# Kingsford-Group/squid

Hardware: AMD Instinct MI355X
Metric: paired-end alignments/sec BAM->_sv.txt (from the BAM files in the page cache: file read, host->device copy, BGZF/BAM decode, graph, ordering, SV calls, _sv.txt written; bit-exact SV calls vs CPU oracle) (higher is better)
Workload: dtype int32

## Files before the change

squid_amd/csrc/sq_inflate_spec.inc:

```
#pragma once
#include "sq_wave.h"

#ifndef SQ_SPEC_PRE
#define SQ_SPEC_PRE 0
#endif
namespace isp {
#ifdef SQ_WAVE_EMU
struct EmuStat { unsigned long long iters = 0, pairs = 0, lits = 0, matches = 0, stretches = 0, max_iters_sum = 0;
    unsigned long long windows = 0, rounds = 0, wave_steps_fix = 0, wave_steps_emit = 0, lane_steps_fix = 0; uint32_t ls[2][64] = {}, le[64] = {};
    void round_done(int par) { uint32_t m = 0; for (int i = 0; i < 64; ++i) { m = ls[par][i] > m ? ls[par][i] : m; lane_steps_fix += ls[par][i]; ls[par][i] = 0; } wave_steps_fix += m; ++rounds; }
    void emit_done() { uint32_t m = 0; for (int i = 0; i < 64; ++i) { m = le[i] > m ? le[i] : m; le[i] = 0; } wave_steps_emit += m; ++windows; } };
inline EmuStat& emu_stat() { static EmuStat s; return s; }
inline int& emu_par_of(int lane) { static int p[64] = {}; return p[lane]; }
#define emu_par() emu_par_of(wv::lane())
#define ISP_STAT(x) x
#else
#define ISP_STAT(x)
#endif

constexpr uint32_t E_VAL = 8, E_XOFF = 17, E_XB = 24, E_NL = 28, E_LIT1 = 1u << 28, E_LIT2 = 2u << 28, E_MATCH = 1u << 30, E_SUB = 1u << 31;
template <int PB> struct Enough;
template <> struct Enough<9> { static constexpr int LL = 852; };
template <> struct Enough<10> { static constexpr int LL = 1334; };
template <> struct Enough<11> { static constexpr int LL = 2342; };
constexpr int DD_PB = 8, DD_N = 402;
constexpr uint32_t OUT_EOB = 1u << 30, OUT_BAD = 1u << 31, OUT_POS = (1u << 30) - 1;

template <int CH, int PB>
struct Lay {
    static constexpr int LL_N = Enough<PB>::LL;
    static constexpr int WIN_DW = (64 * CH / 32 + 16 < 368 ? 368 : 64 * CH / 32 + 16);
    static constexpr int WIN = 0, LENS = WIN, LL = WIN_DW, DD = LL + ((LL_N + 3) & ~3), CLT = DD, MISC = DD + ((DD_N + 3) & ~3), END = MISC + 16;
    static constexpr int BYTES = END * 4;
};
static inline __host__ __device__ uint32_t tok_cap_spec(uint32_t isize, uint32_t clen) { return ((isize >> 1) + (clen >> 3) + 256u + 3u) & ~3u; }

struct Src { const uint32_t* w; uint32_t lim_dw; };
WV_FN uint32_t src_ld(const Src& s, uint32_t d) { return d < s.lim_dw ? s.w[d] : 0u; }
WV_FN unsigned long long src_peek64(const Src& s, uint32_t pos) {
    const uint32_t d = pos >> 5, w0 = src_ld(s, d), w1 = src_ld(s, d + 1), w2 = src_ld(s, d + 2);
    return ((unsigned long long)wv::alignbit(w2, w1, pos) << 32) | wv::alignbit(w1, w0, pos);
}
WV_FN uint32_t ll_entry(int sym, int len) {
    if (sym < 256) return (uint32_t)len | E_LIT1 | ((uint32_t)sym << E_VAL);
    if (sym == 256) return (uint32_t)len;
    const int ls = sym - 257;
    if (ls >= 29) return 0u;
    const uint32_t lx = ls < 8 || ls == 28 ? 0u : (uint32_t)(ls - 4) >> 2;
    const uint32_t lbase = ls < 8 ? 3u + (uint32_t)ls : (ls == 28 ? 258u : 3u + ((4u + ((uint32_t)ls & 3u)) << lx));
    return ((uint32_t)len + lx) | (lbase << E_VAL) | (((uint32_t)len + 2u) << E_XOFF) | (lx << E_XB) | E_MATCH;
}
WV_FN uint32_t dd_entry(int sym, int len) {
    if (sym >= 30) return 0u;
    const uint32_t dx = sym < 4 ? 0u : (uint32_t)(sym - 2) >> 1;
    const uint32_t dbase = sym < 4 ? 1u + (uint32_t)sym : 1u + ((2u + ((uint32_t)sym & 1u)) << dx);
    return ((uint32_t)len + dx) | (dbase << E_VAL) | (dx << E_XB);
}

template <bool IS_LL, int PBITS, int N, int ROUNDS>
WV_FN bool build_table(wv::lds_u32* tbl, const wv::lds_u8* lens, int nsym, wv::lds_u32* alloc_word) {
    const int lane = wv::lane();
    for (int q = lane; q < N; q += 64) tbl[q] = 0u;
    if (lane == 0) *alloc_word = 0u;
    int mylen[ROUNDS];
    uint32_t cnt[16];
#pragma unroll
    for (int l = 0; l < 16; ++l) cnt[l] = 0;
#pragma unroll
// ... 58 lines not shown
        for (int r = 0; r < ROUNDS; ++r) {
            const int l = mylen[r];
            if (l > PBITS) {
                const uint32_t rv = mycode[r], link = tbl[rv & ((1u << PBITS) - 1u)];
                if (link & E_SUB) {
                    const uint32_t nb = (link >> E_XB) & 15u, base = ((link >> E_VAL) & 0xffffu) >> 2;
                    const uint32_t ent = IS_LL ? ll_entry(r * 64 + lane, l) : dd_entry(r * 64 + lane, l);
                    for (uint32_t k = rv >> PBITS; k < (1u << nb); k += 1u << (l - PBITS)) tbl[base + k] = ent;
                }
            }
        }
        wv::sync();
        if (wv::any(!ok)) return false;
    }
    if (IS_LL) {
        for (int i = lane; i < (1 << PBITS); i += 64) {
            const uint32_t e1 = tbl[i];
            if ((e1 >> E_NL) == 1u) {
                const uint32_t cl1 = e1 & 0xffu;
                if (cl1 < (uint32_t)PBITS) {
                    const uint32_t e2 = tbl[(uint32_t)i >> cl1], nl2 = (e2 >> E_NL) & 3u;
                    if (nl2 && !(e2 & (E_SUB | E_MATCH))) {
                        const uint32_t cl2 = nl2 == 2u ? (e2 >> E_XB) & 15u : e2 & 0xffu;
                        if (cl1 + cl2 <= (uint32_t)PBITS) tbl[i] = (cl1 + cl2) | (((e1 >> E_VAL) & 0xffu) << E_VAL) | (((e2 >> E_VAL) & 0xffu) << (E_VAL + 8)) | (cl1 << E_XB) | E_LIT2;
                    }
                }
            }
        }
        wv::sync();
    }
    return true;
}

template <int MODE, int PB>
WV_FN void scan_stretch(const wv::lds_u8* ll, const wv::lds_u8* dd, const wv::lds_u8* win_q , uint32_t start, uint32_t lim,
                        uint32_t* tk , uint32_t at , uint32_t& out, uint32_t& ntok) {
    uint32_t q = start - 2u, nt = at, lit = 0, nlit = 0, status = 0;
    const uint32_t limq = lim - 2u;
    while (q < limq) {
        const wv::lds_u8* wp = win_q + ((q >> 5) << 2);
        const uint32_t w0 = *(const wv::lds_u32*)wp, w1 = *(const wv::lds_u32*)(wp + 4), w2 = *(const wv::lds_u32*)(wp + 8);
        const uint32_t lo = wv::alignbit(w1, w0, q);
        uint32_t e = *(const wv::lds_u32*)(ll + (lo & (((1u << PB) - 1u) << 2)));
        if ((int32_t)e < 0) e = *(const wv::lds_u32*)(ll + ((e >> E_VAL) & 0xffffu) + (wv::bfe(lo, PB + 2, (e >> E_XB) & 15u) << 2));
        const uint32_t nl = (e >> E_NL) & 3u, tot = e & 0xffu, q0 = q;
        ISP_STAT(if (MODE == 2) { ++emu_stat().iters; emu_stat().lits += nl; emu_stat().pairs += nl == 2; emu_stat().matches += e >= E_MATCH; ++emu_stat().le[wv::lane()]; } else ++emu_stat().ls[emu_par()][wv::lane()];)
        q += tot;
        if (MODE) {
            if (MODE == 2) lit |= (nl ? (e >> E_VAL) & 0xffffu : 0u) << (8u * nlit);
            nlit += nl;
            if (nlit >= 3u) {
                if (MODE == 2) { tk[nt] = (lit & 0xffffffu) | (3u << 24); lit >>= 24; }
                ++nt; nlit -= 3u;
            }
        }
        if (e >= E_MATCH) {
            if (MODE) { if (nlit) { if (MODE == 2) { tk[nt] = lit | (nlit << 24); lit = 0; } ++nt; nlit = 0; } }
            const uint32_t hi = wv::alignbit(w2, w1, q0);
            const unsigned long long rest = (((unsigned long long)hi << 32) | lo) >> tot;
            const uint32_t rlo = (uint32_t)rest;
            uint32_t d = *(const wv::lds_u32*)(dd + (rlo & (((1u << DD_PB) - 1u) << 2)));
            if ((int32_t)d < 0) d = *(const wv::lds_u32*)(dd + ((d >> E_VAL) & 0xffffu) + (wv::bfe(rlo, DD_PB + 2, (d >> E_XB) & 15u) << 2));
            if (d == 0u) { status = OUT_BAD; break; }
            q += d & 0xffu;
            if (MODE == 2) {
                const uint32_t len = ((e >> E_VAL) & 0x1ffu) + wv::bfe(lo, (e >> E_XOFF) & 31u, (e >> E_XB) & 15u);
                const uint32_t dxb = (d >> E_XB) & 15u, dist = ((d >> E_VAL) & 0xffffu) + wv::bfe(rlo, (d & 0xffu) - dxb + 2u, dxb);
                tk[nt] = 0x80000000u | (len << 16) | (dist - 1u);
            }
            if (MODE) ++nt;
        } else if (nl == 0u) {
            status = e ? OUT_EOB : OUT_BAD;
            break;
        }
    }
    if (MODE) { if (nlit) { if (MODE == 2) tk[nt] = lit | (nlit << 24); ++nt; } }
    out = (q + 2u) | status;
    ntok = nt - at;
}

struct NoProf { WV_FN void tick(int) {} WV_FN void count(int, uint32_t = 1) {} WV_FN void finish() {} };
template <int CH, int PB, class PROF = NoProf>
WV_FN uint32_t inflate_block_spec(wv::lds_u32* L, const uint8_t* payload, uint32_t clen, uint32_t* tk, uint32_t tcap, bool& err, PROF prof_in = PROF()) {
    PROF prof = prof_in;
    typedef Lay<CH, PB> Y;
    const int lane = wv::lane();
    const uint32_t off0 = (uint32_t)((uintptr_t)payload & 15u);
    Src S{(const uint32_t*)(payload - off0), ((off0 + clen + 15u) >> 4 << 2) + 4u};
    const uint32_t end_bit = (off0 + clen) * 8u;
    wv::lds_u32 *ll = L + Y::LL, *dd = L + Y::DD, *win = L + Y::WIN, *clt = L + Y::CLT, *misc = L + Y::MISC;
    const wv::lds_u8 *llb = (const wv::lds_u8*)ll, *ddb = (const wv::lds_u8*)dd;
    wv::lds_u8* lens = (wv::lds_u8*)(L + Y::LENS);
    uint32_t P = off0 * 8u, nt = 0;
    bool bad = false;
    for (;;) {
        if (P + 3u > end_bit) { bad = true; break; }
        prof.tick(5); prof.count(8);
        unsigned long long h = src_peek64(S, P);
        const uint32_t last = (uint32_t)h & 1u, type = ((uint32_t)h >> 1) & 3u;
        if (type == 3u) { bad = true; break; }
        if (type == 0u) {
            P = (P + 3u + 7u) & ~7u;
            h = src_peek64(S, P);
            const uint32_t len = (uint32_t)h & 0xffffu, nlen = ((uint32_t)h >> 16) & 0xffffu;
            P += 32u;
            if ((len ^ 0xffffu) != nlen || P + len * 8u > end_bit) { bad = true; break; }
            const uint32_t n3 = (len + 2u) / 3u;
            if (nt + n3 > tcap) { bad = true; break; }
            const uint8_t* b = (const uint8_t*)S.w + (P >> 3);
            for (uint32_t i = (uint32_t)lane; i < n3; i += 64u) {
                const uint32_t m = len - 3u * i < 3u ? len - 3u * i : 3u;
                uint32_t t = m << 24;
                for (uint32_t q = 0; q < m; ++q) t |= (uint32_t)b[3u * i + q] << (8u * q);
                tk[nt + i] = t;
            }
            nt += n3; P += len * 8u;
            if (last) break;
// ... 124 lines not shown
                    prev_window = mown ? wv::bcast(last, 63 - wv::clz64(mown)) : prev_window;
                    if (S0c - hd0 * 32u > 8192u) { bad = true; break; }
                }
                wv::sync();
            }
            if (bad) break;
            wv::sync();
            if (lens[256] == 0) { bad = true; break; }
        }
        if (P > end_bit) { bad = true; break; }
        prof.tick(0);
        if (!build_table<true, PB, Y::LL_N, 5>(ll, lens, nlen, misc)) { bad = true; break; }
        if (!build_table<false, DD_PB, DD_N, 1>(dd, lens + nlen, ndist, misc + 1)) { bad = true; break; }
        prof.tick(1);
        uint32_t S0 = P;
        bool in_block = true;
        while (in_block) {
            const uint32_t wd0 = ((S0 - 2u) >> 5) & ~3u;
            const wv::lds_u8* win_q = (const wv::lds_u8*)win - 4u * wd0;
            for (int q = lane; q < Y::WIN_DW / 4; q += 64) {
                const uint32_t d = wd0 + 4u * (uint32_t)q;
                wv::u32x4 v{0u, 0u, 0u, 0u};
                if (d < S.lim_dw) v = wv::load16(S.w + d);
                win[4 * q] = v.x; win[4 * q + 1] = v.y; win[4 * q + 2] = v.z; win[4 * q + 3] = v.w;
            }
            wv::sync();
            prof.tick(2); prof.count(6);
            const uint32_t lim = S0 + (uint32_t)(lane + 1) * (uint32_t)CH;
            uint32_t start = S0 + (uint32_t)lane * (uint32_t)CH, out = 0, mynt = 0;
#if SQ_SPEC_PRE
            if (lane > 0) { uint32_t o0, n0; scan_stretch<0, PB>(llb, ddb, win_q, start - (uint32_t)SQ_SPEC_PRE, start, nullptr, 0u, o0, n0); if (!(o0 & (OUT_EOB | OUT_BAD))) start = o0 & OUT_POS; }
#endif
            uint32_t in_old = start;
            bool dirty = true;
            int E = 63;
            for (;;) {
                prof.count(7);
                if (dirty) scan_stretch<1, PB>(llb, ddb, win_q, start, lim, nullptr, 0u, out, mynt);
                const uint32_t in_new = wv::shfl_up1(out, S0);
                ISP_STAT(if (lane == 0) emu_stat().round_done(emu_par()); emu_par() ^= 1;)
                dirty = false;
                if (lane > 0 && in_new != in_old) {
                    in_old = in_new;
                    if (!(in_new & (OUT_EOB | OUT_BAD))) { start = in_new; dirty = true; }
                }
                const unsigned long long md = wv::ballot(dirty), mend = wv::ballot((out & (OUT_EOB | OUT_BAD)) != 0u);
                const int fd = wv::ctz64(md), fe = wv::ctz64(mend);
                if (fe < fd) { E = fe; break; }
                if (fd == 64) { E = 63; break; }
            }
            prof.tick(3);
            const uint32_t outE = wv::bcast(out, E);
            if (outE & OUT_BAD) { bad = true; break; }
            if ((outE & OUT_POS) > end_bit) { bad = true; break; }
            const uint32_t cntv = lane <= E ? mynt : 0u, incl = wv::scan_incl_add(cntv), total = wv::bcast(incl, 63);
            if (nt + total > tcap) { bad = true; break; }
            if (lane <= E) { uint32_t o2, n2; scan_stretch<2, PB>(llb, ddb, win_q, start, lim, tk, nt + (incl - cntv), o2, n2); }
            nt += total;
            ISP_STAT(wv::sync(); if (lane == 0) emu_stat().emit_done();)
            prof.tick(4);
            if (outE & OUT_EOB) { in_block = false; P = outE & OUT_POS; } else S0 = outE & OUT_POS;
            wv::sync();
        }
        if (bad) break;
        if (last) break;
    }
    prof.tick(5);
    prof.finish();
    err = bad;
    return nt;
}

}
```

squid_amd/csrc/sq_kernels.hip:

```cpp
#include <hip/hip_runtime.h>

#include <algorithm>
#include <atomic>
#include <climits>
#include <cstdio>
#include <cstdlib>
#include <cstring>
#include <functional>
#include <condition_variable>
#include <fcntl.h>
#include <sys/stat.h>
#include <unistd.h>

#include <zlib.h>

#include "sq_internal.h"
#include "sq_inflate_spec.inc"
#include "sq_resolve.inc"
#include "sq_chim_stage.inc"
#include "sq_bwa_stage.inc"
#include "sq_bwa_edges.inc"
#include "sq_bwa_nodes.inc"
#include "sq_segment_stage.inc"
#include "sq_compress_stage.inc"
// ... 2206 lines not shown
        }
        tick(3);
        if (done || sym < 0) continue;
        if (nlit) { push(lit | ((uint32_t)nlit << 24)); lit = 0; nlit = 0; }
        if (sym == 256) { in_block = false; if (last) done = true; continue; }
        const int ls = sym - 257;
        if (ls >= 29) { err = true; done = true; continue; }
        t2_refill(b, ahead);
        const uint32_t lx = ls < 8 || ls == 28 ? 0u : (uint32_t)(ls - 4) >> 2;
        const uint32_t lbase = ls < 8 ? 3u + (uint32_t)ls : (ls == 28 ? 258u : 3u + ((4u + ((uint32_t)ls & 3u)) << lx));
        const uint32_t len = lbase + ((uint32_t)b.buf & ((1u << lx) - 1));
        b.buf >>= lx; b.cnt -= (int)lx;
        int dl;
        const int dat = t2_slot(b, lp_dd, L.k_dd, lane, dl);
        const int ds = dat < 0 ? -1 : (int)L.sym_dd[(dat & 31) * 64 + lane];
        if (ds < 0 || ds >= 30) { err = true; done = true; continue; }
        const uint32_t dx = ds < 4 ? 0u : (uint32_t)(ds - 2) >> 1;
        const uint32_t dbase = ds < 4 ? 1u + (uint32_t)ds : 1u + ((2u + ((uint32_t)ds & 1u)) << dx);
        const uint32_t dist = dbase + ((uint32_t)b.buf & ((1u << dx) - 1));
        b.buf >>= dx; b.cnt -= (int)dx;
        if (dist > outpos || outpos + len > blk.isize) { err = true; done = true; continue; }
        push(0x80000000u | (len << 16) | (dist - 1)); outpos += len;
        tick(4);
    }
    if (PROF && lane == 0) { for (int k = 0; k < 8; ++k) prof[(size_t)blockIdx.x * 8 + k] = pt[k]; }
    if (ntq) { emit(tq0); if (ntq > 1) emit(tq1); if (ntq > 2) emit(tq2); }
    if (have && (err || outpos != blk.isize)) atomicOr(&flags[0], 512);
    if (have) {
        for (uint32_t k = nt - nt % IL_STAGE; k < nt; ++k) tk[k] = stage[(k % IL_STAGE) * 64 + lane];
        ntok[bi] = (int32_t)nt;
    }
}

template <int CH, int PB>
__global__ __launch_bounds__(64) void k_inflate_spec(const uint8_t* file, const InflBlock* blocks, int nblocks, int32_t* flags, uint32_t* tok, int32_t* ntok) {
    extern __shared__ uint32_t isp_lds[];
    const int bi = (int)blockIdx.x;
    if (bi >= nblocks) return;
    const InflBlock blk = blocks[bi];
    bool err = false;
    uint32_t nt = 0;
    if (blk.isize) nt = isp::inflate_block_spec<CH, PB>((wv::lds_u32*)isp_lds, file + blk.coff, blk.clen, tok + blk.toff, isp::tok_cap_spec(blk.isize, blk.clen), err);
    if (threadIdx.x == 0) { ntok[bi] = (int32_t)nt; if (err) atomicOr(&flags[0], 512); }
}
struct SpecProf {
    unsigned long long* g; unsigned long long t0; unsigned long long c[9];
    __device__ SpecProf(unsigned long long* g_) : g(g_), t0(__builtin_amdgcn_s_memtime()) { for (int i = 0; i < 9; ++i) c[i] = 0; }
    __device__ __forceinline__ void tick(int k) { const unsigned long long now = __builtin_amdgcn_s_memtime(); c[k] += now - t0; t0 = now; }
    __device__ __forceinline__ void count(int k, uint32_t n = 1) { c[k] += n; }
    __device__ __forceinline__ void finish() { if ((threadIdx.x & 63u) == 0) for (int i = 0; i < 9; ++i) atomicAdd(&g[i], c[i]); }
};
template <int CH, int PB>
__global__ __launch_bounds__(64) void k_inflate_spec_prof(const uint8_t* file, const InflBlock* blocks, int nblocks, int32_t* flags, uint32_t* tok, int32_t* ntok, unsigned long long* prof) {
    extern __shared__ uint32_t isp_lds[];
    const int bi = (int)blockIdx.x;
    if (bi >= nblocks) return;
    const InflBlock blk = blocks[bi];
    bool err = false;
    uint32_t nt = 0;
    if (blk.isize) nt = isp::inflate_block_spec<CH, PB, SpecProf>((wv::lds_u32*)isp_lds, file + blk.coff, blk.clen, tok + blk.toff, isp::tok_cap_spec(blk.isize, blk.clen), err, SpecProf(prof));
    if (threadIdx.x == 0) { ntok[bi] = (int32_t)nt; if (err) atomicOr(&flags[0], 512); }
}
#ifndef SQ_SPEC_CH
#define SQ_SPEC_CH 384
#endif
#ifndef SQ_SPEC_PB
#define SQ_SPEC_PB 10
#endif
constexpr int SPEC_CH = SQ_SPEC_CH, SPEC_PB = SQ_SPEC_PB;
template <int CH, int PB>
static void launch_inflate_spec(hipStream_t s, const uint8_t* file, const InflBlock* blocks, int nb, int32_t* flags, uint32_t* tok, int32_t* ntok) {
    typedef isp::Lay<CH, PB> Y;
    hipLaunchKernelGGL((k_inflate_spec<CH, PB>), dim3(nb), dim3(64), (size_t)Y::BYTES, s, file, blocks, nb, flags, tok, ntok);
}

__device__ __forceinline__ uint32_t wave_scan_incl(uint32_t x) {
    x += (uint32_t)__builtin_amdgcn_update_dpp(0, (int)x, 0x111, 0xf, 0xf, false);
    x += (uint32_t)__builtin_amdgcn_update_dpp(0, (int)x, 0x112, 0xf, 0xf, false);
    x += (uint32_t)__builtin_amdgcn_update_dpp(0, (int)x, 0x114, 0xf, 0xf, false);
    x += (uint32_t)__builtin_amdgcn_update_dpp(0, (int)x, 0x118, 0xf, 0xf, false);
    x += (uint32_t)__builtin_amdgcn_update_dpp(0, (int)x, 0x142, 0xa, 0xf, false);
    x += (uint32_t)__builtin_amdgcn_update_dpp(0, (int)x, 0x143, 0xc, 0xf, false);
    return x;
}
__global__ __launch_bounds__(128) void k_lz_resolve2(const uint32_t* tok, const int32_t* ntok, const InflBlock* blocks, int nblocks, unsigned long long out_base, uint8_t* outbuf, int32_t* flags) {
    extern __shared__ uint8_t lz_win[];
    __shared__ uint32_t s_base[2];
    __shared__ int s_bad;
    const int lane = threadIdx.x & 63, wave = threadIdx.x >> 6;
    const InflBlock blk = blocks[blockIdx.x];
    const uint32_t* t = tok + blk.toff;
    const int n = ntok[blockIdx.x];
    const int nr = (n + 63) / 64;
    if (threadIdx.x == 0) { s_base[0] = 0; s_base[1] = 0; s_bad = 0; }
    __syncthreads();
    uint32_t nxt = wave * 64 + lane < n ? t[wave * 64 + lane] : 0;
    uint32_t o = 0, len = 0, dist = 1, src = 0, ready_at = 0;
    bool pending = false;
    for (int step = 0; step <= nr; ++step) {
        const bool bad_now = s_bad != 0;
        if (!bad_now && step < nr && (step & 1) == wave) {
            const int r0 = step * 64;
            const uint32_t tk = nxt;
            const int i = r0 + lane;
            if (i + 128 < n) nxt = t[i + 128];
            const bool valid = i < n, is_m = valid && (tk >> 31);
// ... 901 lines not shown
        if (n0 == 0) D.nm_bytes = 0;
        { EvTimer t(c, "k_names", (double)n_rec * 48.0, s);
          hipLaunchKernelGGL(k_name_len, grid_for(n_rec, 256), dim3(256), 0, s, d_bam, d_off, n_rec, D.parse_nblk.p);
          HIPCHK((device_scan<OpSum, true>(s, n_rec, FArrN{D.parse_nblk.p}, D.parse_rel.p, spine, tot))); }
        int32_t nm_total = 0;
        HIPCHK(hipMemcpyAsync(&nm_total, tot, 4, hipMemcpyDeviceToHost, s));
        HIPCHK(hipStreamSynchronize(s));
        if (D.nm_bytes + (size_t)nm_total >= 0xffffffffull) return fail(c, SQ_E_CAPACITY, "more than 4 GB of read names");
        HIPCHK(D.nm_blob.grow_keep(D.nm_bytes, std::max<size_t>(D.nm_bytes + (size_t)nm_total + 64, rec_want * 16), s));
        HIPCHK(D.nm_off.grow_keep(n0, rec_want + 1, s));
        hipLaunchKernelGGL(k_name_copy, grid_for(n_rec, 256), dim3(256), 0, s, d_bam, d_off, n_rec, D.parse_rel.p, (uint32_t)D.nm_bytes, D.nm_blob.p, D.nm_off.p + n0);
        HIPCHK(hipStreamSynchronize(s));
        D.nm_bytes += (size_t)nm_total;
    }
    D.n = (int64_t)n1;
    D.nb = (int64_t)nb1;
    c->counts.n_concordant = D.n;
    c->counts.n_blocks = D.nb;
    return SQ_OK;
}

int dev_token_bench(sq_ctx* c, const char* path, int variant, int max_blocks, int reps, int check, double* out) {
    HIPCHK(hipSetDevice(c->P.device));
    FILE* f = std::fopen(path, "rb");
    if (!f) return fail(c, SQ_E_IO, std::string("cannot open ") + path);
    std::vector<uint8_t> raw;
    std::vector<InflBlock> tab;
    unsigned long long uoff = 0;
    const bool spec = variant != 2;
    for (int b = 0; b < max_blocks; ++b) {
        uint8_t h[18];
        if (std::fread(h, 1, 18, f) != 18) break;
        const size_t bsize = (size_t)(h[16] | (h[17] << 8)) + 1;
        const size_t at = raw.size();
        raw.resize(at + bsize);
        std::memcpy(raw.data() + at, h, 18);
        if (std::fread(raw.data() + at + 18, 1, bsize - 18, f) != bsize - 18) { raw.resize(at); break; }
        uint32_t isize; std::memcpy(&isize, raw.data() + at + bsize - 4, 4);
        tab.push_back(InflBlock{at + 18, (uint32_t)(bsize - 26), isize, uoff, 0});
        uoff += isize;
    }
    std::fclose(f);
    if (tab.empty()) return fail(c, SQ_E_IO, "no BGZF block read");
    unsigned long long slots = 0;
    for (InflBlock& ib : tab) { ib.toff = slots; slots += spec ? isp::tok_cap_spec(ib.isize, ib.clen) : t2_tok_cap(ib.isize); }
    const int nb = (int)tab.size();
    DBuf<uint8_t> d_in, d_out; DBuf<InflBlock> d_tab; DBuf<uint32_t> d_tok, d_lens; DBuf<int32_t> d_ntok, d_flags;
    struct Rel { DBuf<uint8_t>&a, &b; DBuf<InflBlock>& t; DBuf<uint32_t>&k, &l; DBuf<int32_t>&n, &fl; ~Rel() { a.release(); b.release(); t.release(); k.release(); l.release(); n.release(); fl.release(); } } rel{d_in, d_out, d_tab, d_tok, d_lens, d_ntok, d_flags};
    HIPCHK(d_in.reserve(raw.size() + 512)); HIPCHK(d_out.reserve((size_t)uoff + 512)); HIPCHK(d_tab.reserve((size_t)nb)); HIPCHK(d_tok.reserve((size_t)slots + 64));
    HIPCHK(d_ntok.reserve((size_t)nb)); HIPCHK(d_flags.reserve(16)); HIPCHK(d_lens.reserve(((size_t)nb + 128) * T2_LENS_WORDS));
    HIPCHK(hipMemcpy(d_in.p, raw.data(), raw.size(), hipMemcpyHostToDevice));
    HIPCHK(hipMemcpy(d_tab.p, tab.data(), (size_t)nb * sizeof(InflBlock), hipMemcpyHostToDevice));
    HIPCHK(hipMemset(d_flags.p, 0, 64));
    HIPCHK(hipFuncSetAttribute((const void*)k_inflate_tok2<false>, hipFuncAttributeMaxDynamicSharedMemorySize, 5 * (int)T2_LDS_BYTES));
    hipStream_t s = c->stream;
    hipEvent_t e0, e1, e2;
    HIPCHK(hipEventCreate(&e0)); HIPCHK(hipEventCreate(&e1)); HIPCHK(hipEventCreate(&e2));
    double tok_ms = 0, res_ms = 0;
    for (int r = 0; r < reps + 1; ++r) {
        HIPCHK(hipEventRecord(e0, s));
        switch (variant) {
            case 2: hipLaunchKernelGGL(k_inflate_tok2<false>, dim3((nb + 63) / 64), dim3(64), T2_LDS_BYTES, s, d_in.p, d_tab.p, nb, d_flags.p, d_tok.p, d_ntok.p, d_lens.p, nullptr); break;
            case 51211: launch_inflate_spec<512, 11>(s, d_in.p, d_tab.p, nb, d_flags.p, d_tok.p, d_ntok.p); break;
            case 51210: launch_inflate_spec<512, 10>(s, d_in.p, d_tab.p, nb, d_flags.p, d_tok.p, d_ntok.p); break;
            case 25610: launch_inflate_spec<256, 10>(s, d_in.p, d_tab.p, nb, d_flags.p, d_tok.p, d_ntok.p); break;
            case 25611: launch_inflate_spec<256, 11>(s, d_in.p, d_tab.p, nb, d_flags.p, d_tok.p, d_ntok.p); break;
            case 38411: launch_inflate_spec<384, 11>(s, d_in.p, d_tab.p, nb, d_flags.p, d_tok.p, d_ntok.p); break;
            case 38410: launch_inflate_spec<384, 10>(s, d_in.p, d_tab.p, nb, d_flags.p, d_tok.p, d_ntok.p); break;
            case 32010: launch_inflate_spec<320, 10>(s, d_in.p, d_tab.p, nb, d_flags.p, d_tok.p, d_ntok.p); break;
            case 19210: launch_inflate_spec<192, 10>(s, d_in.p, d_tab.p, nb, d_flags.p, d_tok.p, d_ntok.p); break;
            case 102411: launch_inflate_spec<1024, 11>(s, d_in.p, d_tab.p, nb, d_flags.p, d_tok.p, d_ntok.p); break;
            case 25609: launch_inflate_spec<256, 9>(s, d_in.p, d_tab.p, nb, d_flags.p, d_tok.p, d_ntok.p); break;
            case 12809: launch_inflate_spec<128, 9>(s, d_in.p, d_tab.p, nb, d_flags.p, d_tok.p, d_ntok.p); break;
            case 12810: launch_inflate_spec<128, 10>(s, d_in.p, d_tab.p, nb, d_flags.p, d_tok.p, d_ntok.p); break;
            case 51209: launch_inflate_spec<512, 9>(s, d_in.p, d_tab.p, nb, d_flags.p, d_tok.p, d_ntok.p); break;
            default: return fail(c, SQ_E_ARG, "unknown token pass variant");
        }
        HIPCHK(hipEventRecord(e1, s));
        if (resolve_staged()) hipLaunchKernelGGL(k_lz_resolve5, dim3(nb), dim3(64), 0, s, d_tok.p, d_ntok.p, d_tab.p, nb, 0ull, d_out.p, d_flags.p + 4);
        else hipLaunchKernelGGL(k_lz_resolve3, dim3(nb), dim3(64), 0, s, d_tok.p, d_ntok.p, d_tab.p, nb, 0ull, d_out.p, d_flags.p + 4);
        HIPCHK(hipEventRecord(e2, s));
        HIPCHK(hipStreamSynchronize(s));
        float a = 0, b = 0;
        HIPCHK(hipEventElapsedTime(&a, e0, e1)); HIPCHK(hipEventElapsedTime(&b, e1, e2));
        if (r) { tok_ms += a; res_ms += b; }
    }
    (void)hipEventDestroy(e0); (void)hipEventDestroy(e1); (void)hipEventDestroy(e2);
    if (variant == 51211 || variant == 25610) {
        DBuf<unsigned long long> d_prof;
        HIPCHK(d_prof.reserve(16)); HIPCHK(hipMemset(d_prof.p, 0, 16 * 8));
        if (variant == 51211) { typedef isp::Lay<512, 11> Y; hipLaunchKernelGGL((k_inflate_spec_prof<512, 11>), dim3(nb), dim3(64), (size_t)Y::BYTES, s, d_in.p, d_tab.p, nb, d_flags.p, d_tok.p, d_ntok.p, d_prof.p); }
        else { typedef isp::Lay<256, 10> Y; hipLaunchKernelGGL((k_inflate_spec_prof<256, 10>), dim3(nb), dim3(64), (size_t)Y::BYTES, s, d_in.p, d_tab.p, nb, d_flags.p, d_tok.p, d_ntok.p, d_prof.p); }
        unsigned long long pr[9];
        HIPCHK(hipStreamSynchronize(s));
        HIPCHK(hipMemcpy(pr, d_prof.p, sizeof pr, hipMemcpyDeviceToHost));
        d_prof.release();
        double tot = 0; for (int i = 0; i < 6; ++i) tot += (double)pr[i];
        std::fprintf(stderr, "token pass %d, cycles of a block (s_memtime, 100 MHz ticks?): %.0f | headers %.1f %% tables %.1f %% window loads %.1f %% scans %.1f %% token writing %.1f %% rest %.1f %% | per block: %.1f deflate blocks, %.1f windows, %.2f scan rounds per window\n",
                     variant, tot / nb, 100.0 * pr[0] / tot, 100.0 * pr[1] / tot, 100.0 * pr[2] / tot, 100.0 * pr[3] / tot, 100.0 * pr[4] / tot, 100.0 * pr[5] / tot, (double)pr[8] / nb, (double)pr[6] / nb, (double)pr[7] / std::max<double>(1, (double)pr[6]));
    }
    int32_t fl[8];
    HIPCHK(hipMemcpy(fl, d_flags.p, sizeof fl, hipMemcpyDeviceToHost));
    std::vector<int32_t> nt((size_t)nb);
    HIPCHK(hipMemcpy(nt.data(), d_ntok.p, (size_t)nb * 4, hipMemcpyDeviceToHost));
    long long ntok = 0;
    for (int32_t v : nt) ntok += v;
    long bad = (fl[0] | fl[4]) ? -1 : 0;
    if (check && bad == 0) {
        std::vector<uint8_t> got((size_t)uoff), want;
        HIPCHK(hipMemcpy(got.data(), d_out.p, (size_t)uoff, hipMemcpyDeviceToHost));
        for (const InflBlock& b : tab) {
            want.resize(b.isize);
            z_stream zs; std::memset(&zs, 0, sizeof zs);
            inflateInit2(&zs, -15);
            zs.next_in = (Bytef*)(raw.data() + b.coff); zs.avail_in = b.clen; zs.next_out = want.data(); zs.avail_out = b.isize;
            inflate(&zs, Z_FINISH); inflateEnd(&zs);
            if (b.isize && std::memcmp(want.data(), got.data() + b.uoff, b.isize) != 0) ++bad;
        }
    }
    out[0] = tok_ms / std::max(1, reps); out[1] = res_ms / std::max(1, reps); out[2] = (double)uoff; out[3] = (double)raw.size(); out[4] = nb; out[5] = (double)ntok; out[6] = (double)bad;
    return SQ_OK;
}

int dev_ingest_bgzf(sq_ctx* c, const uint8_t* file, std::vector<BgzfRange>& blocks, size_t b0, size_t b1, size_t begin, bool synced, int nref, const IndexMore& index_more_in, size_t file_bytes, GpuFileSrc* src) {
// ... 95 lines not shown
    };
    const unsigned long long first_uoff = blocks[b0].uoff;
    auto range_bytes_estimate = [&]() -> unsigned long long {
        std::lock_guard<std::mutex> lk(bm);
        if (!index_more) { const size_t e = std::min(b1, blocks.size()); return blocks[e - 1].uoff + blocks[e - 1].isize - first_uoff; }
        const BgzfRange &f = blocks.front(), &l = blocks.back();
        const double ratio = (double)(l.uoff + l.isize - f.uoff) / (double)std::max<unsigned long long>(1, l.coff + l.clen - f.coff);
        return (unsigned long long)(ratio * 1.03 * (double)(file_bytes - std::min<unsigned long long>(file_bytes, f.coff)));
    };
    if (tok_spec && !cap_given) {
        unsigned long long est = range_bytes_estimate();
        if (index_more && src && src->stop != (size_t)-1) {
            std::lock_guard<std::mutex> lk(bm);
            const BgzfRange &f = blocks.front(), &l = blocks.back();
            const double ratio = (double)(l.uoff + l.isize - f.uoff) / (double)std::max<unsigned long long>(1, l.coff + l.clen - f.coff);
            if (src->stop > f.coff) est = (unsigned long long)(ratio * 1.03 * (double)(std::min<unsigned long long>(src->stop, file_bytes) - f.coff));
        }
        cap = std::max<unsigned long long>((unsigned long long)64 << 20, std::min(cap, est / 24));
    }
    Shard sh_here = c->shard;
    if (c->capture_names) sh_here.on = false;
    const Shard& sh = sh_here;
    auto stage_a = [&](size_t k) -> int {
        if (!plan(k)) return SQ_OK;
        const Batch B = batches[k];
        { const int rc = ensure_set((int)(k % (size_t)D.il_depth)); if (rc) return fail(c, rc, "cannot create the stream of a buffer set"); }
        DeviceRecords::InflSet& st = D.il_set[k % (size_t)D.il_depth];
        hipStream_t sa = D.il_stream[k % (size_t)D.il_depth];
        const int nb = (int)(B.end - B.at);
        st.host_tab.resize((size_t)nb);
        for (int i = 0; i < nb; ++i) { const BgzfRange& b = blocks[B.at + (size_t)i]; st.host_tab[(size_t)i] = InflBlock{b.coff - B.coff0, b.clen, b.isize, b.uoff, 0}; }
        std::stable_sort(st.host_tab.begin(), st.host_tab.end(), [](const InflBlock& x, const InflBlock& y) { return x.clen > y.clen; });
        unsigned long long tok_slots = 0;
        for (InflBlock& ib : st.host_tab) { ib.toff = tok_slots; tok_slots += tok_spec ? isp::tok_cap_spec(ib.isize, ib.clen) : t2_tok_cap(ib.isize); }
        const auto wa0 = std::chrono::steady_clock::now();
        const unsigned long long full = std::max<unsigned long long>(B.bbytes, std::min<unsigned long long>(cap, range_bytes_estimate()));
        const double cratio = (double)B.cbytes / (double)std::max<unsigned long long>(B.bbytes, 1);
        const uint8_t* dfile = c->ingest_dfile ? c->ingest_dfile : (feed ? feed->dfile() : nullptr);
        if (!dfile) HIPCHK(st.in.reserve(std::max((size_t)B.cbytes, (size_t)(cratio * 1.1 * (double)full)) + 256));
        st.src = dfile ? dfile + B.coff0 : st.in.p;
        HIPCHK(st.tab.reserve(std::max((size_t)nb, (size_t)(full / 60000)))); HIPCHK(st.flags.reserve(4));
        const size_t tok_full = tok_spec ? (size_t)(full / 2 + (unsigned long long)(cratio * 1.1 * (double)full) / 8 + 260 * (full / 60000 + 1)) : (size_t)(full / 2 + 80 * (full / 60000 + 1));
        HIPCHK(st.tok.reserve(std::max((size_t)tok_slots, tok_full) + 64)); HIPCHK(st.ntok.reserve(std::max((size_t)nb, (size_t)(full / 60000))));
        if (!tok_spec) HIPCHK(st.lens.reserve((std::max((size_t)nb, (size_t)(full / 60000)) + 128) * T2_LENS_WORDS));
        const double wa1 = since_ms(wa0);
        if (!dfile) {
            if (k >= (size_t)D.il_depth) HIPCHK(hipEventSynchronize(st.ready));
            const int rc = h2d_parallel(c, st.in.p, file + B.coff0, (size_t)B.cbytes);
            if (rc) return rc;
        }
        const double wa2 = since_ms(wa0);
        if (feed) { const int rc = feed->wait_bytes((size_t)B.coff0, (size_t)(B.coff0 + B.cbytes) + 256, sa); if (rc) return rc; }
        const double wa3 = since_ms(wa0);
        struct Rep { bool on; size_t k; double at, a1, a2, a3, gb; std::chrono::steady_clock::time_point t0; ~Rep() { if (on) std::fprintf(stderr, "GPU ingest: batch %zu planned at %.1f ms, buffers %.1f ms, copy of %.2f GB returned after %.1f ms, its pieces queued after %.1f ms, table + token pass queued after %.1f ms\n", k, at, a1, gb, a2 - a1, a3 - a2, std::chrono::duration<double, std::milli>(std::chrono::steady_clock::now() - t0).count() - a3); } }
            rep{report && k < 3, k, std::chrono::duration<double, std::milli>(wa0 - w0).count(), wa1, wa2, wa3, (double)B.cbytes * 1e-9, wa0};
        HIPCHK(hipMemcpyAsync(st.tab.p, st.host_tab.data(), (size_t)nb * sizeof(InflBlock), hipMemcpyHostToDevice, sa));
        HIPCHK(hipMemsetAsync(st.flags.p, 0, 4 * 4, sa));
        if (tok_spec) {
            EvTimer t1(c, "k_inflate_spec", (double)B.cbytes + (double)B.bbytes * 2, sa);
            launch_inflate_spec<SPEC_CH, SPEC_PB>(sa, st.src, st.tab.p, nb, st.flags.p, st.tok.p, st.ntok.p);
        } else {
            EvTimer t1(c, "k_inflate_tok2", (double)B.cbytes + (double)B.bbytes * 2, sa);
            hipLaunchKernelGGL(k_inflate_tok2<false>, dim3(((nb + 63) / 64 + tok_wpb - 1) / tok_wpb), dim3(64 * tok_wpb), tok_wpb * T2_LDS_BYTES, sa, st.src, st.tab.p, nb, st.flags.p, st.tok.p, st.ntok.p, st.lens.p, nullptr);
        }
        DeviceRecords::PostSet& P = D.il_post[k % (size_t)D.il_depth];
        HIPCHK(P.out.reserve((size_t)room + (size_t)full + ((size_t)1 << 20) + 64));
        if (k >= (size_t)D.il_depth) HIPCHK(hipStreamWaitEvent(sa, P.carried, 0));
        {
            EvTimer t2(c, resolve_global ? (resolve_staged() ? "k_lz_resolve5" : "k_lz_resolve3") : "k_lz_resolve2", (double)B.bbytes * 3, sa);
            if (resolve_global && resolve_staged()) hipLaunchKernelGGL(k_lz_resolve5, dim3(nb), dim3(64), 0, sa, st.tok.p, st.ntok.p, st.tab.p, nb, B.bbase, P.out.p + room, st.flags.p);
            else if (resolve_global) hipLaunchKernelGGL(k_lz_resolve3, dim3(nb), dim3(64), 0, sa, st.tok.p, st.ntok.p, st.tab.p, nb, B.bbase, P.out.p + room, st.flags.p);
            else hipLaunchKernelGGL(k_lz_resolve2, dim3(nb), dim3(128), 65536 + 16, sa, st.tok.p, st.ntok.p, st.tab.p, nb, B.bbase, P.out.p + room, st.flags.p);
        }
        HIPCHK(hipEventRecord(st.ready, sa));
        return SQ_OK;
// ... 1503 lines not shown
```

Baseline: 341.9 million.

## Stage speculative inflate tokens per lane and copy instead of re-decoding

The speculative inflate fix-up loop now writes tokens into a per-lane global staging area (SC slots per lane, placed after each block's token capacity) during re-scans, with a first pass that only counts. When every lane's token count fits in its staging slots, the emit step copies the staged tokens to their final offsets instead of running a third Huffman decode pass. Otherwise it falls back to the old emit scan. This trades extra global writes and a larger token buffer for skipping one decode pass per window. It also adds a BGZF header check and event cleanup in the benchmark path.

Measured after the change: 341.0 million. No clear change (-0.3%).

```diff
diff --git a/squid_amd/csrc/sq_inflate_spec.inc b/squid_amd/csrc/sq_inflate_spec.inc
--- a/squid_amd/csrc/sq_inflate_spec.inc
+++ b/squid_amd/csrc/sq_inflate_spec.inc
@@ -7,8 +7,12 @@
 namespace isp {
 #ifdef SQ_WAVE_EMU
 struct EmuStat { unsigned long long iters = 0, pairs = 0, lits = 0, matches = 0, stretches = 0, max_iters_sum = 0;
-    unsigned long long windows = 0, rounds = 0, wave_steps_fix = 0, wave_steps_emit = 0, lane_steps_fix = 0; uint32_t ls[2][64] = {}, le[64] = {};
-    void round_done(int par) { uint32_t m = 0; for (int i = 0; i < 64; ++i) { m = ls[par][i] > m ? ls[par][i] : m; lane_steps_fix += ls[par][i]; ls[par][i] = 0; } wave_steps_fix += m; ++rounds; }
+    unsigned long long windows = 0, rounds = 0, wave_steps_fix = 0, wave_steps_stage = 0, wave_steps_emit = 0, lane_steps_fix = 0; uint32_t ls[2][64] = {}, le[64] = {}, lw[2][64] = {};
+    unsigned long long fallback_windows = 0, moved = 0, hist[257] = {};
+    void round_done(int par) {
+        uint32_t m = 0, mw = 0;
+        for (int i = 0; i < 64; ++i) { m = ls[par][i] > m ? ls[par][i] : m; lane_steps_fix += ls[par][i]; ls[par][i] = 0; mw = lw[par][i] > mw ? lw[par][i] : mw; lw[par][i] = 0; }
+        wave_steps_fix += m; wave_steps_stage += mw; ++rounds; }
     void emit_done() { uint32_t m = 0; for (int i = 0; i < 64; ++i) { m = le[i] > m ? le[i] : m; le[i] = 0; } wave_steps_emit += m; ++windows; } };
 inline EmuStat& emu_stat() { static EmuStat s; return s; }
 inline int& emu_par_of(int lane) { static int p[64] = {}; return p[lane]; }
@@ -33,7 +37,9 @@
     static constexpr int WIN = 0, LENS = WIN, LL = WIN_DW, DD = LL + ((LL_N + 3) & ~3), CLT = DD, MISC = DD + ((DD_N + 3) & ~3), END = MISC + 16;
     static constexpr int BYTES = END * 4;
 };
-static inline __host__ __device__ uint32_t tok_cap_spec(uint32_t isize, uint32_t clen) { return ((isize >> 1) + (clen >> 3) + 256u + 3u) & ~3u; }
+constexpr int spec_sc(int CH) { return (CH / 12 + 4 + 3) & ~3; }
+static inline __host__ __device__ uint32_t tok_final_cap(uint32_t isize, uint32_t clen) { return ((isize >> 1) + (clen >> 3) + 256u + 3u) & ~3u; }
+static inline __host__ __device__ uint32_t tok_cap_spec(uint32_t isize, uint32_t clen, int sc) { return tok_final_cap(isize, clen) + 64u * (uint32_t)sc; }
 
 struct Src { const uint32_t* w; uint32_t lim_dw; };
 WV_FN uint32_t src_ld(const Src& s, uint32_t d) { return d < s.lim_dw ? s.w[d] : 0u; }
@@ -158,11 +164,12 @@
     return true;
 }
 
-template <int MODE, int PB>
+template <int MODE, int PB, int CAP = 0>
 WV_FN void scan_stretch(const wv::lds_u8* ll, const wv::lds_u8* dd, const wv::lds_u8* win_q , uint32_t start, uint32_t lim,
                         uint32_t* tk , uint32_t at , uint32_t& out, uint32_t& ntok) {
     uint32_t q = start - 2u, nt = at, lit = 0, nlit = 0, status = 0;
     const uint32_t limq = lim - 2u;
+    auto put = [&](uint32_t v) { if (MODE == 2 || nt < at + (uint32_t)CAP) tk[nt] = v; };
     while (q < limq) {
         const wv::lds_u8* wp = win_q + ((q >> 5) << 2);
         const uint32_t w0 = *(const wv::lds_u32*)wp, w1 = *(const wv::lds_u32*)(wp + 4), w2 = *(const wv::lds_u32*)(wp + 8);
@@ -170,18 +177,18 @@
         uint32_t e = *(const wv::lds_u32*)(ll + (lo & (((1u << PB) - 1u) << 2)));
         if ((int32_t)e < 0) e = *(const wv::lds_u32*)(ll + ((e >> E_VAL) & 0xffffu) + (wv::bfe(lo, PB + 2, (e >> E_XB) & 15u) << 2));
         const uint32_t nl = (e >> E_NL) & 3u, tot = e & 0xffu, q0 = q;
-        ISP_STAT(if (MODE == 2) { ++emu_stat().iters; emu_stat().lits += nl; emu_stat().pairs += nl == 2; emu_stat().matches += e >= E_MATCH; ++emu_stat().le[wv::lane()]; } else ++emu_stat().ls[emu_par()][wv::lane()];)
+        ISP_STAT(if (MODE == 3) ++emu_stat().lw[emu_par()][wv::lane()]; else if (MODE == 2) { ++emu_stat().iters; emu_stat().lits += nl; emu_stat().pairs += nl == 2; emu_stat().matches += e >= E_MATCH; ++emu_stat().le[wv::lane()]; } else ++emu_stat().ls[emu_par()][wv::lane()];)
         q += tot;
         if (MODE) {
-            if (MODE == 2) lit |= (nl ? (e >> E_VAL) & 0xffffu : 0u) << (8u * nlit);
+            if (MODE >= 2) lit |= (nl ? (e >> E_VAL) & 0xffffu : 0u) << (8u * nlit);
             nlit += nl;
             if (nlit >= 3u) {
-                if (MODE == 2) { tk[nt] = (lit & 0xffffffu) | (3u << 24); lit >>= 24; }
+                if (MODE >= 2) { put((lit & 0xffffffu) | (3u << 24)); lit >>= 24; }
                 ++nt; nlit -= 3u;
             }
         }
         if (e >= E_MATCH) {
-            if (MODE) { if (nlit) { if (MODE == 2) { tk[nt] = lit | (nlit << 24); lit = 0; } ++nt; nlit = 0; } }
+            if (MODE) { if (nlit) { if (MODE >= 2) { put(lit | (nlit << 24)); lit = 0; } ++nt; nlit = 0; } }
             const uint32_t hi = wv::alignbit(w2, w1, q0);
             const unsigned long long rest = (((unsigned long long)hi << 32) | lo) >> tot;
             const uint32_t rlo = (uint32_t)rest;
@@ -189,10 +196,10 @@
             if ((int32_t)d < 0) d = *(const wv::lds_u32*)(dd + ((d >> E_VAL) & 0xffffu) + (wv::bfe(rlo, DD_PB + 2, (d >> E_XB) & 15u) << 2));
             if (d == 0u) { status = OUT_BAD; break; }
             q += d & 0xffu;
-            if (MODE == 2) {
+            if (MODE >= 2) {
                 const uint32_t len = ((e >> E_VAL) & 0x1ffu) + wv::bfe(lo, (e >> E_XOFF) & 31u, (e >> E_XB) & 15u);
                 const uint32_t dxb = (d >> E_XB) & 15u, dist = ((d >> E_VAL) & 0xffffu) + wv::bfe(rlo, (d & 0xffu) - dxb + 2u, dxb);
-                tk[nt] = 0x80000000u | (len << 16) | (dist - 1u);
+                put(0x80000000u | (len << 16) | (dist - 1u));
             }
             if (MODE) ++nt;
         } else if (nl == 0u) {
@@ -200,15 +207,17 @@
             break;
         }
     }
-    if (MODE) { if (nlit) { if (MODE == 2) tk[nt] = lit | (nlit << 24); ++nt; } }
+    if (MODE) { if (nlit) { if (MODE >= 2) put(lit | (nlit << 24)); ++nt; } }
     out = (q + 2u) | status;
     ntok = nt - at;
 }
 
 struct NoProf { WV_FN void tick(int) {} WV_FN void count(int, uint32_t = 1) {} WV_FN void finish() {} };
-template <int CH, int PB, class PROF = NoProf>
-WV_FN uint32_t inflate_block_spec(wv::lds_u32* L, const uint8_t* payload, uint32_t clen, uint32_t* tk, uint32_t tcap, bool& err, PROF prof_in = PROF()) {
+template <int CH, int PB, int SC = spec_sc(CH), class PROF = NoProf>
+WV_FN uint32_t inflate_block_spec(wv::lds_u32* L, const uint8_t* payload, uint32_t clen, uint32_t* tk, uint32_t tcap_all, bool& err, PROF prof_in = PROF()) {
     PROF prof = prof_in;
+    const uint32_t tcap = tcap_all - 64u * (uint32_t)SC;
+    uint32_t* const stage = tk + tcap;
     typedef Lay<CH, PB> Y;
     const int lane = wv::lane();
     const uint32_t off0 = (uint32_t)((uintptr_t)payload & 15u);
@@ -399,11 +408,13 @@
             if (lane > 0) { uint32_t o0, n0; scan_stretch<0, PB>(llb, ddb, win_q, start - (uint32_t)SQ_SPEC_PRE, start, nullptr, 0u, o0, n0); if (!(o0 & (OUT_EOB | OUT_BAD))) start = o0 & OUT_POS; }
 #endif
             uint32_t in_old = start;
-            bool dirty = true;
+            bool dirty = true, first = true;
             int E = 63;
             for (;;) {
                 prof.count(7);
-                if (dirty) scan_stretch<1, PB>(llb, ddb, win_q, start, lim, nullptr, 0u, out, mynt);
+                if constexpr (SC == 0) { if (dirty) scan_stretch<1, PB>(llb, ddb, win_q, start, lim, nullptr, 0u, out, mynt); }
+                else if (first) scan_stretch<0, PB>(llb, ddb, win_q, start, lim, nullptr, 0u, out, mynt);
+                else if (dirty) scan_stretch<3, PB, SC>(llb, ddb, win_q, start, lim, stage, (uint32_t)(lane * SC), out, mynt);
                 const uint32_t in_new = wv::shfl_up1(out, S0);
                 ISP_STAT(if (lane == 0) emu_stat().round_done(emu_par()); emu_par() ^= 1;)
                 dirty = false;
@@ -411,6 +422,8 @@
                     in_old = in_new;
                     if (!(in_new & (OUT_EOB | OUT_BAD))) { start = in_new; dirty = true; }
                 }
+                if (SC != 0 && first && !(in_new & (OUT_EOB | OUT_BAD))) dirty = true;
+                first = false;
                 const unsigned long long md = wv::ballot(dirty), mend = wv::ballot((out & (OUT_EOB | OUT_BAD)) != 0u);
                 const int fd = wv::ctz64(md), fe = wv::ctz64(mend);
                 if (fe < fd) { E = fe; break; }
@@ -422,7 +435,31 @@
             if ((outE & OUT_POS) > end_bit) { bad = true; break; }
             const uint32_t cntv = lane <= E ? mynt : 0u, incl = wv::scan_incl_add(cntv), total = wv::bcast(incl, 63);
             if (nt + total > tcap) { bad = true; break; }
-            if (lane <= E) { uint32_t o2, n2; scan_stretch<2, PB>(llb, ddb, win_q, start, lim, tk, nt + (incl - cntv), o2, n2); }
+            ISP_STAT(if (lane <= E) ++emu_stat().hist[mynt < 256u ? mynt : 256u];)
+            bool staged = false;
+            if constexpr (SC != 0) staged = !wv::any(cntv > (uint32_t)SC);
+            if (!staged) {
+                ISP_STAT(if (lane == 0 && SC != 0) ++emu_stat().fallback_windows;)
+                if (lane <= E) { uint32_t o2, n2; scan_stretch<2, PB>(llb, ddb, win_q, start, lim, tk, nt + (incl - cntv), o2, n2); }
+            } else if constexpr (SC != 0) {
+                const uint32_t* src = stage + lane * SC;
+                uint32_t* dst = tk + nt + (incl - cntv);
+                ISP_STAT(emu_stat().moved += cntv;)
+#pragma unroll
+                for (int k0 = 0; k0 < SC; k0 += 8) {
+                    if (!wv::any((uint32_t)k0 < cntv)) break;
+                    uint32_t v[8];
+                    if (SC % 4 == 0) {
+#pragma unroll
+                        for (int k = 0; k < 8; k += 4) if (k0 + k < SC) { const wv::u32x4 t = wv::load16(src + k0 + k); v[k] = t.x; v[k + 1] = t.y; v[k + 2] = t.z; v[k + 3] = t.w; }
+                    } else {
+#pragma unroll
+                        for (int k = 0; k < 8; ++k) if (k0 + k < SC) v[k] = src[k0 + k];
+                    }
+#pragma unroll
+                    for (int k = 0; k < 8; ++k) if (k0 + k < SC && (uint32_t)(k0 + k) < cntv) dst[k0 + k] = v[k];
+                }
+            }
             nt += total;
             ISP_STAT(wv::sync(); if (lane == 0) emu_stat().emit_done();)
             prof.tick(4);
diff --git a/squid_amd/csrc/sq_kernels.hip b/squid_amd/csrc/sq_kernels.hip
--- a/squid_amd/csrc/sq_kernels.hip
+++ b/squid_amd/csrc/sq_kernels.hip
@@ -2262,7 +2262,7 @@
     }
 }
 
-template <int CH, int PB>
+template <int CH, int PB, int SC = isp::spec_sc(CH)>
 __global__ __launch_bounds__(64) void k_inflate_spec(const uint8_t* file, const InflBlock* blocks, int nblocks, int32_t* flags, uint32_t* tok, int32_t* ntok) {
     extern __shared__ uint32_t isp_lds[];
     const int bi = (int)blockIdx.x;
@@ -2270,7 +2270,7 @@
     const InflBlock blk = blocks[bi];
     bool err = false;
     uint32_t nt = 0;
-    if (blk.isize) nt = isp::inflate_block_spec<CH, PB>((wv::lds_u32*)isp_lds, file + blk.coff, blk.clen, tok + blk.toff, isp::tok_cap_spec(blk.isize, blk.clen), err);
+    if (blk.isize) nt = isp::inflate_block_spec<CH, PB, SC>((wv::lds_u32*)isp_lds, file + blk.coff, blk.clen, tok + blk.toff, isp::tok_cap_spec(blk.isize, blk.clen, SC), err);
     if (threadIdx.x == 0) { ntok[bi] = (int32_t)nt; if (err) atomicOr(&flags[0], 512); }
 }
 struct SpecProf {
@@ -2288,7 +2288,7 @@
     const InflBlock blk = blocks[bi];
     bool err = false;
     uint32_t nt = 0;
-    if (blk.isize) nt = isp::inflate_block_spec<CH, PB, SpecProf>((wv::lds_u32*)isp_lds, file + blk.coff, blk.clen, tok + blk.toff, isp::tok_cap_spec(blk.isize, blk.clen), err, SpecProf(prof));
+    if (blk.isize) nt = isp::inflate_block_spec<CH, PB, isp::spec_sc(CH), SpecProf>((wv::lds_u32*)isp_lds, file + blk.coff, blk.clen, tok + blk.toff, isp::tok_cap_spec(blk.isize, blk.clen, isp::spec_sc(CH)), err, SpecProf(prof));
     if (threadIdx.x == 0) { ntok[bi] = (int32_t)nt; if (err) atomicOr(&flags[0], 512); }
 }
 #ifndef SQ_SPEC_CH
@@ -2297,11 +2297,11 @@
 #ifndef SQ_SPEC_PB
 #define SQ_SPEC_PB 10
 #endif
-constexpr int SPEC_CH = SQ_SPEC_CH, SPEC_PB = SQ_SPEC_PB;
-template <int CH, int PB>
+constexpr int SPEC_CH = SQ_SPEC_CH, SPEC_PB = SQ_SPEC_PB, SPEC_SC = isp::spec_sc(SPEC_CH);
+template <int CH, int PB, int SC = isp::spec_sc(CH)>
 static void launch_inflate_spec(hipStream_t s, const uint8_t* file, const InflBlock* blocks, int nb, int32_t* flags, uint32_t* tok, int32_t* ntok) {
     typedef isp::Lay<CH, PB> Y;
-    hipLaunchKernelGGL((k_inflate_spec<CH, PB>), dim3(nb), dim3(64), (size_t)Y::BYTES, s, file, blocks, nb, flags, tok, ntok);
+    hipLaunchKernelGGL((k_inflate_spec<CH, PB, SC>), dim3(nb), dim3(64), (size_t)Y::BYTES, s, file, blocks, nb, flags, tok, ntok);
 }
 
 __device__ __forceinline__ uint32_t wave_scan_incl(uint32_t x) {
@@ -3269,6 +3269,7 @@
         uint8_t h[18];
         if (std::fread(h, 1, 18, f) != 18) break;
         const size_t bsize = (size_t)(h[16] | (h[17] << 8)) + 1;
+        if (h[0] != 31 || h[1] != 139 || h[2] != 8 || h[3] != 4 || h[10] != 6 || h[11] != 0 || h[12] != 'B' || h[13] != 'C' || h[14] != 2 || h[15] != 0 || bsize < 28) { std::fclose(f); return fail(c, SQ_E_IO, std::string("not a BGZF block in ") + path); }
         const size_t at = raw.size();
         raw.resize(at + bsize);
         std::memcpy(raw.data() + at, h, 18);
@@ -3280,7 +3281,8 @@
     std::fclose(f);
     if (tab.empty()) return fail(c, SQ_E_IO, "no BGZF block read");
     unsigned long long slots = 0;
-    for (InflBlock& ib : tab) { ib.toff = slots; slots += spec ? isp::tok_cap_spec(ib.isize, ib.clen) : t2_tok_cap(ib.isize); }
+    const int sc = variant >= 4000000 ? 4 : isp::spec_sc(variant / 100);
+    for (InflBlock& ib : tab) { ib.toff = slots; slots += spec ? isp::tok_cap_spec(ib.isize, ib.clen, sc) : t2_tok_cap(ib.isize); }
     const int nb = (int)tab.size();
     DBuf<uint8_t> d_in, d_out; DBuf<InflBlock> d_tab; DBuf<uint32_t> d_tok, d_lens; DBuf<int32_t> d_ntok, d_flags;
     struct Rel { DBuf<uint8_t>&a, &b; DBuf<InflBlock>& t; DBuf<uint32_t>&k, &l; DBuf<int32_t>&n, &fl; ~Rel() { a.release(); b.release(); t.release(); k.release(); l.release(); n.release(); fl.release(); } } rel{d_in, d_out, d_tab, d_tok, d_lens, d_ntok, d_flags};
@@ -3291,8 +3293,9 @@
     HIPCHK(hipMemset(d_flags.p, 0, 64));
     HIPCHK(hipFuncSetAttribute((const void*)k_inflate_tok2<false>, hipFuncAttributeMaxDynamicSharedMemorySize, 5 * (int)T2_LDS_BYTES));
     hipStream_t s = c->stream;
-    hipEvent_t e0, e1, e2;
-    HIPCHK(hipEventCreate(&e0)); HIPCHK(hipEventCreate(&e1)); HIPCHK(hipEventCreate(&e2));
+    struct Events { hipEvent_t e[3] = {nullptr, nullptr, nullptr}; ~Events() { for (hipEvent_t x : e) if (x) (void)hipEventDestroy(x); } } ev;
+    for (hipEvent_t& x : ev.e) HIPCHK(hipEventCreate(&x));
+    const hipEvent_t e0 = ev.e[0], e1 = ev.e[1], e2 = ev.e[2];
     double tok_ms = 0, res_ms = 0;
     for (int r = 0; r < reps + 1; ++r) {
         HIPCHK(hipEventRecord(e0, s));
@@ -3311,6 +3314,7 @@
             case 12809: launch_inflate_spec<128, 9>(s, d_in.p, d_tab.p, nb, d_flags.p, d_tok.p, d_ntok.p); break;
             case 12810: launch_inflate_spec<128, 10>(s, d_in.p, d_tab.p, nb, d_flags.p, d_tok.p, d_ntok.p); break;
             case 51209: launch_inflate_spec<512, 9>(s, d_in.p, d_tab.p, nb, d_flags.p, d_tok.p, d_ntok.p); break;
+            case 4000000 + SPEC_CH * 100 + SPEC_PB: launch_inflate_spec<SPEC_CH, SPEC_PB, 4>(s, d_in.p, d_tab.p, nb, d_flags.p, d_tok.p, d_ntok.p); break;
             default: return fail(c, SQ_E_ARG, "unknown token pass variant");
         }
         HIPCHK(hipEventRecord(e1, s));
@@ -3322,11 +3326,11 @@
         HIPCHK(hipEventElapsedTime(&a, e0, e1)); HIPCHK(hipEventElapsedTime(&b, e1, e2));
         if (r) { tok_ms += a; res_ms += b; }
     }
-    (void)hipEventDestroy(e0); (void)hipEventDestroy(e1); (void)hipEventDestroy(e2);
-    if (variant == 51211 || variant == 25610) {
+    if (variant == 51211 || variant == 25610 || variant == SPEC_CH * 100 + SPEC_PB) {
         DBuf<unsigned long long> d_prof;
         HIPCHK(d_prof.reserve(16)); HIPCHK(hipMemset(d_prof.p, 0, 16 * 8));
-        if (variant == 51211) { typedef isp::Lay<512, 11> Y; hipLaunchKernelGGL((k_inflate_spec_prof<512, 11>), dim3(nb), dim3(64), (size_t)Y::BYTES, s, d_in.p, d_tab.p, nb, d_flags.p, d_tok.p, d_ntok.p, d_prof.p); }
+        if (variant == SPEC_CH * 100 + SPEC_PB) { typedef isp::Lay<SPEC_CH, SPEC_PB> Y; hipLaunchKernelGGL((k_inflate_spec_prof<SPEC_CH, SPEC_PB>), dim3(nb), dim3(64), (size_t)Y::BYTES, s, d_in.p, d_tab.p, nb, d_flags.p, d_tok.p, d_ntok.p, d_prof.p); }
+        else if (variant == 51211) { typedef isp::Lay<512, 11> Y; hipLaunchKernelGGL((k_inflate_spec_prof<512, 11>), dim3(nb), dim3(64), (size_t)Y::BYTES, s, d_in.p, d_tab.p, nb, d_flags.p, d_tok.p, d_ntok.p, d_prof.p); }
         else { typedef isp::Lay<256, 10> Y; hipLaunchKernelGGL((k_inflate_spec_prof<256, 10>), dim3(nb), dim3(64), (size_t)Y::BYTES, s, d_in.p, d_tab.p, nb, d_flags.p, d_tok.p, d_ntok.p, d_prof.p); }
         unsigned long long pr[9];
         HIPCHK(hipStreamSynchronize(s));
@@ -3488,7 +3492,7 @@
         for (int i = 0; i < nb; ++i) { const BgzfRange& b = blocks[B.at + (size_t)i]; st.host_tab[(size_t)i] = InflBlock{b.coff - B.coff0, b.clen, b.isize, b.uoff, 0}; }
         std::stable_sort(st.host_tab.begin(), st.host_tab.end(), [](const InflBlock& x, const InflBlock& y) { return x.clen > y.clen; });
         unsigned long long tok_slots = 0;
-        for (InflBlock& ib : st.host_tab) { ib.toff = tok_slots; tok_slots += tok_spec ? isp::tok_cap_spec(ib.isize, ib.clen) : t2_tok_cap(ib.isize); }
+        for (InflBlock& ib : st.host_tab) { ib.toff = tok_slots; tok_slots += tok_spec ? isp::tok_cap_spec(ib.isize, ib.clen, SPEC_SC) : t2_tok_cap(ib.isize); }
         const auto wa0 = std::chrono::steady_clock::now();
         const unsigned long long full = std::max<unsigned long long>(B.bbytes, std::min<unsigned long long>(cap, range_bytes_estimate()));
         const double cratio = (double)B.cbytes / (double)std::max<unsigned long long>(B.bbytes, 1);
@@ -3496,7 +3500,7 @@
         if (!dfile) HIPCHK(st.in.reserve(std::max((size_t)B.cbytes, (size_t)(cratio * 1.1 * (double)full)) + 256));
         st.src = dfile ? dfile + B.coff0 : st.in.p;
         HIPCHK(st.tab.reserve(std::max((size_t)nb, (size_t)(full / 60000)))); HIPCHK(st.flags.reserve(4));
-        const size_t tok_full = tok_spec ? (size_t)(full / 2 + (unsigned long long)(cratio * 1.1 * (double)full) / 8 + 260 * (full / 60000 + 1)) : (size_t)(full / 2 + 80 * (full / 60000 + 1));
+        const size_t tok_full = tok_spec ? (size_t)(full / 2 + (unsigned long long)(cratio * 1.1 * (double)full) / 8 + (260 + 64 * SPEC_SC) * (full / 60000 + 1)) : (size_t)(full / 2 + 80 * (full / 60000 + 1));
         HIPCHK(st.tok.reserve(std::max((size_t)tok_slots, tok_full) + 64)); HIPCHK(st.ntok.reserve(std::max((size_t)nb, (size_t)(full / 60000))));
         if (!tok_spec) HIPCHK(st.lens.reserve((std::max((size_t)nb, (size_t)(full / 60000)) + 128) * T2_LENS_WORDS));
         const double wa1 = since_ms(wa0);
```
